# chungongyu/siga

Measured on AMD Instinct MI355X. Metric: reads/sec overlapped (ASQG bit-exact), higher is better.
Workload: dtype u64

## Files before the change

siga_amd/csrc/sigax_kernels.hip:

```cpp
#include <hip/hip_runtime.h>

#include <cstdlib>

#include "sigax_kernels.h"

typedef unsigned long long u64;
typedef unsigned int u32;

#ifndef SIGAX_NT
#define SIGAX_NT 7
#endif

struct Cnt4 {
  u64 a, c, g, t;
};

template <bool WIDE> struct PosOf { typedef u32 type; };
template <> struct PosOf<true> { typedef u64 type; };
template <typename P> struct Cnt4P {
  P a, c, g, t;
};

template <bool WIDE> struct Cand;
template <> struct __attribute__((aligned(32))) Cand<false> {
// ... 170 lines not shown
      "global_load_dwordx4 %3, %9, %12 offset:48\n\t"
      "global_load_dwordx4 %5, %10, %12 offset:16\n\t"
      "global_load_dwordx4 %6, %10, %12 offset:32\n\t"
      "global_load_dwordx4 %7, %10, %12 offset:48\n\t"
      "s_waitcnt vmcnt(0)"
      : "=&v"(a.k0), "=&v"(a.k1), "=&v"(a.k2), "=&v"(a.k3), "=&v"(b.k0), "=&v"(b.k1), "=&v"(b.k2), "=&v"(b.k3), "=&v"(ch)
      : "v"(offa), "v"(offb), "v"(offc), "s"(gbase), "s"(sbase)
      : "memory");
}
__device__ __forceinline__ void find_step_loads8(const void* qa, const void* qb, Gran& a, Gran& b) {
  asm volatile(
      "global_load_dwordx4 %0, %8, off\n\t"
      "global_load_dwordx4 %4, %9, off\n\t"
      "global_load_dwordx4 %1, %8, off offset:16\n\t"
      "global_load_dwordx4 %2, %8, off offset:32\n\t"
      "global_load_dwordx4 %3, %8, off offset:48\n\t"
      "global_load_dwordx4 %5, %9, off offset:16\n\t"
      "global_load_dwordx4 %6, %9, off offset:32\n\t"
      "global_load_dwordx4 %7, %9, off offset:48\n\t"
      "s_waitcnt vmcnt(0)"
      : "=&v"(a.k0), "=&v"(a.k1), "=&v"(a.k2), "=&v"(a.k3), "=&v"(b.k0), "=&v"(b.k1), "=&v"(b.k2), "=&v"(b.k3)
      : "v"(qa), "v"(qb)
      : "memory");
}
__device__ __forceinline__ void find_step_loads8_s(const void* gbase, u32 offa, u32 offb, Gran& a, Gran& b) {
  asm volatile(
      "global_load_dwordx4 %0, %8, %10\n\t"
      "global_load_dwordx4 %4, %9, %10\n\t"
      "global_load_dwordx4 %1, %8, %10 offset:16\n\t"
      "global_load_dwordx4 %2, %8, %10 offset:32\n\t"
      "global_load_dwordx4 %3, %8, %10 offset:48\n\t"
      "global_load_dwordx4 %5, %9, %10 offset:16\n\t"
      "global_load_dwordx4 %6, %9, %10 offset:32\n\t"
      "global_load_dwordx4 %7, %9, %10 offset:48\n\t"
      "s_waitcnt vmcnt(0)"
      : "=&v"(a.k0), "=&v"(a.k1), "=&v"(a.k2), "=&v"(a.k3), "=&v"(b.k0), "=&v"(b.k1), "=&v"(b.k2), "=&v"(b.k3)
      : "v"(offa), "v"(offb), "s"(gbase)
      : "memory");
}
__device__ __forceinline__ void chunk_count(const v4u& k, int take, u32& a, u32& c, u32& g, u32& t) {
  u32 m = take >= 32 ? 0xFFFFFFFFu : (take <= 0 ? 0u : ((1u << take) - 1u));
  u32 x0 = k.y & m, x1 = k.z & m, x2 = k.w & m;
  a += __popc(x0 & ~x1);
  c += __popc(x1 & ~x0);
  g += __popc(x0 & x1);
  t += __popc(x2);
}
template <bool WIDE>
__device__ __forceinline__ Cnt4P<typename PosOf<WIDE>::type> fm_rank4p_from(const FmRef& s, u64 pc, const Gran& q) {
  typedef typename PosOf<WIDE>::type P;
  int r = (int)(pc & 127u);
  u32 a = q.k0.x, c = q.k1.x, g = q.k2.x, t = q.k3.x;
  chunk_count(q.k0, r, a, c, g, t);
  chunk_count(q.k1, r - 32, a, c, g, t);
  chunk_count(q.k2, r - 64, a, c, g, t);
  chunk_count(q.k3, r - 96, a, c, g, t);
  Cnt4P<P> o;
  o.a = a; o.c = c; o.g = g; o.t = t;
  if (WIDE) {
    const u64* sb = s.super + (pc >> SIGAX_SUPER_SHIFT) * 4;
    o.a += (P)sb[0]; o.c += (P)sb[1]; o.g += (P)sb[2]; o.t += (P)sb[3];
  }
  return o;
}

__device__ __forceinline__ u32 fm_char(const FmRef& s, u64 i) {
  const u32* q = reinterpret_cast<const u32*>(s.g) + (i >> 7) * 16 + ((i >> 5) & 3) * 4;
  u32 b = (u32)i & 31u;
  return ((q[1] >> b) & 1u) | (((q[2] >> b) & 1u) << 1) | (((q[3] >> b) & 1u) << 2);
}

__device__ __forceinline__ u32 base_rank(u32 ch) {
  const u32 i = (ch >> 1) & 3u;
  const u32 expect = (0x47544341u >> (i * 8)) & 0xFFu;
  const u32 rank = (0x3421u >> (i * 4)) & 0xFu;
  return expect == ch ? rank : 0u;
}
template <typename T>
__device__ __forceinline__ T sel5(u32 r, T v0, T v1, T v2, T v3, T v4) {
  const bool b0 = (r & 1u) != 0, b1 = (r & 2u) != 0, b2 = (r & 4u) != 0;
  const T t01 = b0 ? v1 : v0, t23 = b0 ? v3 : v2;
  const T t = b1 ? t23 : t01;
  return b2 ? v4 : t;
}
__device__ __forceinline__ u32 comp_rank(u32 r) { return r ? 5u - r : 0u; }

__device__ __forceinline__ u64 wave_sum(u64 v) {
  for (int off = 32; off > 0; off >>= 1) v += __shfl_xor(v, off, 64);
  return v;
}

template <bool WIDE>
__global__ __launch_bounds__(256) void k_occ_batch(FmStrand s, const u64* pos, u64 n, u64* out) {
  u64 i = (u64)blockIdx.x * 256 + threadIdx.x;
  if (i >= n) return;
  u64 v[5];
  fm_rank5<WIDE>(fm_ref(s, 0), pos[i] + 1, v);
  for (int k = 0; k < 5; ++k) out[i * 5 + k] = v[k];
}

template <bool WIDE>
__global__ __launch_bounds__(256) void k_kmer_count(FmStrand s, const unsigned char* kmers, u32 k, u64 n, u64* out) {
  u64 i = (u64)blockIdx.x * 256 + threadIdx.x;
  if (i >= n) return;
  const unsigned char* w = kmers + i * k;
  FmRef f = fm_ref(s, 0);
  u64 C[5] = {s.C[0], s.C[1], s.C[2], s.C[3], s.C[4]};
  u64 T[5] = {s.total[0], s.total[1], s.total[2], s.total[3], s.total[4]};
  auto sel = [](const u64 v[5], u32 r) { return r == 0 ? v[0] : r == 1 ? v[1] : r == 2 ? v[2] : r == 3 ? v[3] : v[4]; };
  u32 r = base_rank(w[k - 1]);
  u64 lo = sel(C, r), hi = lo + sel(T, r) - 1;
  for (u32 j = k - 1; j > 0; --j) {
    if (!(hi != ~0ull && hi >= lo)) break;
    r = base_rank(w[j - 1]);
    u64 l[5], u[5];
    fm_rank5<WIDE>(f, lo, l);
    fm_rank5<WIDE>(f, hi + 1, u);
    lo = sel(C, r) + sel(l, r);
    hi = sel(C, r) + sel(u, r) - 1;
  }
  out[i] = (hi != ~0ull && hi >= lo) ? hi - lo + 1 : 0;
}

template <bool WIDE>
__device__ __forceinline__ u32 lf_row(const FmRef& f, const u64* C, u64 p, u64* next) {
  const u32 c = fm_char(f, p);
  const Cnt4 k = fm_rank<WIDE>(f, p);
  if (c == 0) *next = p - (k.a + k.c + k.g + k.t);
  else *next = C[c] + (c == 1 ? k.a : c == 2 ? k.c : c == 3 ? k.g : k.t);
  return c;
}
#define STRETCH_BAD (~0ull)
template <bool WIDE>
__global__ __launch_bounds__(256) void k_stretch_scan(FmStrand s, u64 n_stretch, u64* info, u32* maxlen) {
  const u64 j = (u64)blockIdx.x * 256 + threadIdx.x;
  u32 mine = 0;
  if (j < n_stretch) {
    const FmRef f = fm_ref(s, 0);
    const u64 C[5] = {s.C[0], s.C[1], s.C[2], s.C[3], s.C[4]};
    u64 p = j, len = 0, v = STRETCH_BAD;
    for (;;) {
      u64 q;
      if (lf_row<WIDE>(f, C, p, &q) == 0) { v = (len << 32) | (q & 0xFFFFFFFFull); break; }
      p = q;
      if (++len >= s.n || len >= (1ull << 28)) { len = 0; break; }
    }
    info[j] = v;
    mine = (u32)len;
  }
  for (int off = 32; off > 0; off >>= 1) mine = max(mine, (u32)__shfl_xor((int)mine, off, 64));
  if ((threadIdx.x & 63u) == 0 && mine) atomicMax(maxlen, mine);
}
__device__ __forceinline__ void packed_or(unsigned char* tab, u64 p, u32 bits, u64 v) {
  const u64 B = p * bits;
  u64* w = reinterpret_cast<u64*>(tab) + (B >> 6);
  const u32 sh = (u32)B & 63u;
  atomicOr(w, v << sh);
  if (sh + bits > 64u) atomicOr(w + 1, v >> (64u - sh));
}
__device__ __forceinline__ u64 packed_get(const unsigned char* tab, u64 p, u32 bits) {
  const u64 B = p * bits;
  u64 v;
#if (SIGAX_NT & 1)
  {
    typedef u64 __attribute__((aligned(1))) u64u;
    v = __builtin_nontemporal_load(reinterpret_cast<const u64u*>(tab + (B >> 3)));
// ... 363 lines not shown
  asm volatile(
      "global_load_dwordx4 %0, %11, %15" SIGAX_FIND_POLICY "\n\t"
      "global_load_dwordx4 %1, %12, %15" SIGAX_FIND_POLICY "\n\t"
      "global_load_dwordx4 %2, %11, %15 offset:80" SIGAX_FIND_POLICY "\n\t"
      "global_load_dwordx4 %3, %11, %15 offset:96" SIGAX_FIND_POLICY "\n\t"
      "global_load_dwordx4 %4, %11, %15 offset:112" SIGAX_FIND_POLICY "\n\t"
      "s_and_saveexec_b64 %10, %16\n\t"
      "global_load_dwordx4 %5, %13, %15" SIGAX_FIND_POLICY "\n\t"
      "global_load_dwordx4 %6, %14, %15" SIGAX_FIND_POLICY "\n\t"
      "global_load_dwordx4 %7, %13, %15 offset:80" SIGAX_FIND_POLICY "\n\t"
      "global_load_dwordx4 %8, %13, %15 offset:96" SIGAX_FIND_POLICY "\n\t"
      "global_load_dwordx4 %9, %13, %15 offset:112" SIGAX_FIND_POLICY "\n\t"
      "s_mov_b64 exec, %10\n\t"
      "s_waitcnt vmcnt(0)"
      : "=&v"(a.s), "=&v"(a.pc), "=&v"(a.p5), "=&v"(a.p6), "=&v"(a.p7), "=&v"(b.s), "=&v"(b.pc), "=&v"(b.p5), "=&v"(b.p6),
        "=&v"(b.p7), "=&s"(saved)
      : "v"(offa), "v"(offa_c), "v"(offb), "v"(offb_c), "s"(base), "s"(two)
      : "memory", "scc");
}
#define COOP_A_U4 512u
#define COOP_B_U4 128u
#define COOP_WAVE_U4 (COOP_A_U4 + COOP_B_U4 + 16u)
__device__ __forceinline__ void find_step2_dma(const uint32_t* gran2, u32 la, u32 lb, u32 c, uint4* stage, u32 lane, Gran2& a, Gran2& b) {
  const u32 j = lane & 7u, pp = lane >> 3;
  const char* base = reinterpret_cast<const char*>(gran2);
  u32* list = reinterpret_cast<u32*>(stage + COOP_A_U4 + COOP_B_U4);
  const bool differ = lb != la;
  const u64 dmask = __ballot(differ);
  const u32 nd = (u32)__popcll(dmask);
  const u32 r = (u32)__popcll(dmask & ((1ull << lane) - 1ull));
  asm volatile("s_waitcnt lgkmcnt(0)" ::: "memory");
  if (differ) list[r] = lb;
#pragma unroll
  for (u32 t = 0; t < 8; ++t) {
    const u32 lA = (u32)__shfl((int)la, (int)(8u * t + j), 64);
    const u32 p = pp ^ (t & 1u);
    const char* sa = base + (u64)lA * 128u + p * 16u;
    __builtin_amdgcn_global_load_lds((const __attribute__((address_space(1))) void*)sa,
                                     (__attribute__((address_space(3))) void*)(u32)(size_t)(stage + t * 64u), 16, 0, 0);
  }
  const u32 tt = lane >> 3, x = tt & 1u;
  auto ld = [](const uint4* q) { const uint4 v = *q; v4u w; w.x = v.x; w.y = v.y; w.z = v.z; w.w = v.w; return w; };
  bool gotA = false;
  const u32 npass = (nd + 15u) >> 4;
  for (u32 ps = 0; ps < npass || !gotA; ++ps) {
    if (ps < npass) {
      asm volatile("s_waitcnt lgkmcnt(0)" ::: "memory");
      __builtin_amdgcn_fence(__ATOMIC_ACQ_REL, "wavefront");
      __builtin_amdgcn_wave_barrier();
#pragma unroll
      for (u32 t = 0; t < 2; ++t) {
        const u32 rk = 16u * ps + 8u * t + j;
        if (rk < nd) {
          const u32 lB = list[rk];
          const u32 p = pp ^ (t & 1u);
          const char* sb = base + (u64)lB * 128u + p * 16u;
          __builtin_amdgcn_global_load_lds((const __attribute__((address_space(1))) void*)sb,
                                           (__attribute__((address_space(3))) void*)(u32)(size_t)(stage + COOP_A_U4 + t * 64u), 16, 0, 0);
        }
      }
    }
    asm volatile("s_waitcnt vmcnt(0)" ::: "memory");
    __builtin_amdgcn_fence(__ATOMIC_ACQUIRE, "wavefront");
    __builtin_amdgcn_wave_barrier();
    if (!gotA) {
      const uint4* qa = stage + tt * 64u + j;
      a.s = ld(qa + ((0u ^ x) * 8u)); a.pc = ld(qa + ((c ^ x) * 8u)); a.p5 = ld(qa + ((5u ^ x) * 8u)); a.p6 = ld(qa + ((6u ^ x) * 8u)); a.p7 = ld(qa + ((7u ^ x) * 8u));
      gotA = true;
    }
    if (differ && (r >> 4) == ps) {
      const u32 q = r & 15u, tb = q >> 3, xb = tb & 1u;
      const uint4* qb = stage + COOP_A_U4 + tb * 64u + (q & 7u);
      b.s = ld(qb + ((0u ^ xb) * 8u)); b.pc = ld(qb + ((c ^ xb) * 8u)); b.p5 = ld(qb + ((5u ^ xb) * 8u)); b.p6 = ld(qb + ((6u ^ xb) * 8u)); b.p7 = ld(qb + ((7u ^ xb) * 8u));
    }
  }
  asm volatile("s_waitcnt lgkmcnt(0)" ::: "memory");
  if (!differ) b = a;
}

struct Rank2 {
  u32 a, c, g, t;
  u32 pa, pc, pg, pt;
};
__device__ __forceinline__ Rank2 rank2_from(const Gran2& q, u32 r, u32 c) {
  const u32 m0 = r >= 32 ? 0xFFFFFFFFu : ((1u << r) - 1u);
  const u32 m1 = r > 32 ? ((1u << (r - 32)) - 1u) : 0u;
  const bool cb0 = ((c - 1u) & 1u) != 0, cb1 = ((c - 1u) & 2u) != 0;
  Rank2 o;
  o.a = q.s.x; o.c = q.s.y; o.g = q.s.z; o.t = q.s.w;
  o.pa = q.pc.x; o.pc = q.pc.y; o.pg = q.pc.z; o.pt = q.pc.w;
  auto word = [&](u32 y, u32 z, u32 w, u32 y2, u32 z2, u32 w2, u32 m) {
    const u32 A = y & ~z, C = z & ~y, G = y & z, T = w;
    o.a += __popc(A & m); o.c += __popc(C & m); o.g += __popc(G & m); o.t += __popc(T & m);
    const u32 E = (cb1 ? (cb0 ? T : G) : (cb0 ? C : A)) & m;
    o.pa += __popc(y2 & ~z2 & E); o.pc += __popc(z2 & ~y2 & E); o.pg += __popc(y2 & z2 & E); o.pt += __popc(w2 & E);
  };
  word(q.p5.x, q.p5.z, q.p6.x, q.p6.z, q.p7.x, q.p7.z, m0);
  word(q.p5.y, q.p5.w, q.p6.y, q.p6.w, q.p7.y, q.p7.w, m1);
  return o;
}
template <bool WIDE>
struct Find2TablesT {
  typedef typename PosOf<WIDE>::type P;
  P Cc[2][4][4];
  P Cd[2][4];
};
typedef Find2TablesT<false> Find2Tables;
template <bool WIDE>
__device__ __forceinline__ void find2_tables_load(Find2TablesT<WIDE>& t, const FmStrand& fwd, const FmStrand& rev) {
  typedef typename PosOf<WIDE>::type P;
  if (threadIdx.x < 8) {
    const u32 which = threadIdx.x >> 2, c = (threadIdx.x & 3u) + 1u;
    const FmStrand& st = which ? rev : fwd;
    const FmRef F = fm_ref(st, which);
    const u64 pos = st.C[c];
    const Cnt4 k = fm_rank<WIDE>(F, pos);
    t.Cc[which][c - 1][0] = (P)k.a; t.Cc[which][c - 1][1] = (P)k.c; t.Cc[which][c - 1][2] = (P)k.g; t.Cc[which][c - 1][3] = (P)k.t;
    t.Cd[which][c - 1] = (P)(pos - (k.a + k.c + k.g + k.t));
  }
}

template <int NT>
struct FindStageT {
  static constexpr bool direct = false;
  uint4 row_[NT][4];
  u64 tag_[NT];
  __device__ __forceinline__ uint4* row(u32 t) { return row_[t]; }
  __device__ __forceinline__ u64& tag(u32 t) { return tag_[t]; }
};
typedef FindStageT<256> FindStage;
typedef FindStageT<128> FindStageC;
struct FindStageNone {
  static constexpr bool direct = true;
  __device__ __forceinline__ uint4* row(u32) { return nullptr; }
  __device__ __forceinline__ u64& tag(u32) { return dummy; }
  u64 dummy;
};

template <class SG>
__device__ __forceinline__ void find_flush(SG& sg, bool want, u32 tid) {
  if constexpr (SG::direct) return;
  const u32 lane = tid & 63u, q0 = tid & ~3u, piece = tid & 3u;
  __builtin_amdgcn_wave_barrier();
  u64 bal = __ballot(want);
  u32 qm = (u32)(bal >> (lane & 60u)) & 0xFu;
  while (__ballot(qm != 0) != 0) {
    if (qm != 0) {
      const u32 src = q0 + (u32)__builtin_ctz(qm);
      const u64 tag = sg.tag(src);
      if (piece <= (u32)(tag & 3u)) {
        const uint4 v = sg.row(src)[piece];
#if (SIGAX_NT & 2)
        {
          typedef u32 nt4 __attribute__((ext_vector_type(4)));
          nt4 w;
          w.x = v.x; w.y = v.y; w.z = v.z; w.w = v.w;
          __builtin_nontemporal_store(w, reinterpret_cast<nt4*>((tag & ~(u64)3) + piece * 16u));
        }
#else
        *reinterpret_cast<uint4*>((tag & ~(u64)3) + piece * 16u) = v;
#endif
      }
      qm &= qm - 1u;
    }
  }
  __builtin_amdgcn_wave_barrier();
}

__device__ __forceinline__ u32 rd_rank(const unsigned char* rd, u32 i) { return ((u32)rd[i >> 1] >> ((i & 1u) * 4u)) & 15u; }

template <bool WIDE, bool STAGED, bool TWO, bool COOP = false, int NT = 256, class SG = FindStage>
__device__ __forceinline__ void find_body(const FindArgs& A, FmTables& tb, SG& sg, const Find2TablesT<WIDE>& t2,
                                          const unsigned char* rd, u64 rd_base, uint4* coop_stage = nullptr, u32 tile = blockIdx.x) {
  const u32 tid = threadIdx.x;
  const u32 wv = __builtin_amdgcn_readfirstlane(tid >> 6);
  const u32 o = A.chain_base + (wv & (A.chains_per_wg - 1u));
  const u32 wslot = (wv / A.chains_per_wg) * 64u + (tid & 63u);
  const u32 slot = A.read_begin + tile * ((u32)NT / A.chains_per_wg) + wslot;
  const bool inr = slot < A.read_end;
  const u32 read = (A.perm != nullptr && inr) ? A.perm[slot] : slot;
  typedef typename PosOf<WIDE>::type P;
  u32 nocc = 0;
  u32 nsec = 0;
  u32 nb = 0, flagbits = 0;
  bool live = inr && ((A.chain_mask >> o) & 1u);
  u64 b0 = 0;
  u32 L = 0;
  if (live) {
    b0 = A.offs[read];
    L = (u32)(A.offs[read + 1] - b0);
    live = L > 0;
  }
  const bool pf = o < 2;
  const FmRef F = fm_ref(A.fwd, 0), R = fm_ref(A.rev, 1);
  const FmRef PI = fm_pick(pf, F, R);
  const FmRef OI = fm_pick(pf, R, F);
  const u64* CP = tb.C[PI.which];
  const u64* CO = tb.C[OI.which];
  const void* PI2 = pf ? (const void*)A.fwd.gran2 : (const void*)A.rev.gran2;
  const u64* PS2 = pf ? A.fwd.super2 : A.rev.super2;
  const bool comp = (o & 1u) != 0;
  const bool fromStart = (o == 1 || o == 2);
  const u32 af = o == 0 ? SIGAX_AF_CHAIN0 : o == 1 ? SIGAX_AF_CHAIN1 : o == 2 ? SIGAX_AF_CHAIN2 : SIGAX_AF_CHAIN3;
  const unsigned char* sq = A.seqs + b0;
  const u32 rdo = A.perm != nullptr ? wslot * A.stage_stride : (u32)(b0 - rd_base);
  const u64 b0w = ((u64)__builtin_amdgcn_readfirstlane((u32)(b0 >> 32)) << 32) | __builtin_amdgcn_readfirstlane((u32)b0);
  const unsigned char* sq0 = A.seqs + b0w;
  const u32 sqd = (u32)(b0 - b0w);
  auto slot_addr = [&](u32 i) -> u64 {
    return reinterpret_cast<u64>(A.arena) + (((u64)read * 4 + o) * A.cap + i) * sizeof(Cand<WIDE>);
  };

  P lo0 = 0, sz = 0, lo1 = 0;
  u32 s = 1;
  bool started = false;
  if (STAGED && A.deep_k != 0u) {
    const u32 K = A.deep_k;
    const bool can = live && L >= K;
    if (__ballot(can) != 0) {
      u64 k0 = 0, k1 = 0;
      bool acgt = can;
      for (u32 i = 0; i < K; ++i) {
        u32 r = 1u;
        if (can) {
          const u32 at = rdo + (fromStart ? i : L - 1u - i);
          r = COOP ? rd_rank(rd, at) : base_rank(rd[at]);
        }
        if (comp) r = comp_rank(r);
        acgt = acgt && r != 0u;
        const u64 c = (u64)((r - 1u) & 3u);
        if (i < 32u) k0 |= c << (2u * i);
        else k1 |= c << (2u * (i - 32u));
      }
      if (acgt) {
        k1 |= (u64)(0x8000u | K) << 48;
        P a0 = 0, a1 = 0, az = 0;
        if (deep_lookup<WIDE>(pf ? A.fwd.deep : A.rev.deep, pf ? A.fwd.deep_slots : A.rev.deep_slots, k0, k1, a0, a1, az)) {
          lo0 = a0; lo1 = a1; sz = az; s = K;
          started = true;
        }
      }
    }
  }
  if (STAGED && live && !started && A.start_ok && L >= (u32)SIGAX_START_K) {
    const void* ST = pf ? A.fwd.start : A.rev.start;
    u32 code = 0;
    bool acgt = true;
#pragma unroll
    for (u32 i = 0; i < (u32)SIGAX_START_K; ++i) {
      const u32 at = rdo + (fromStart ? i : L - 1u - i);
      u32 r = COOP ? rd_rank(rd, at) : base_rank(rd[at]);
      if (comp) r = comp_rank(r);
      acgt = acgt && r != 0u;
      code = (code << 2) | ((r - 1u) & 3u);
    }
    if (acgt) {
      if (WIDE) {
        const ulonglong2* q = reinterpret_cast<const ulonglong2*>(ST) + 2ull * code;
        const ulonglong2 a = q[0], b = q[1];
        lo0 = (P)a.x; lo1 = (P)a.y; sz = (P)b.x; s = (u32)b.y;
      } else {
        const uint4 e = reinterpret_cast<const uint4*>(ST)[code];
        lo0 = (P)e.x; lo1 = (P)e.y; sz = (P)e.z; s = e.w;
      }
      started = true;
    }
  }
  nsec += (u32)__popcll(__ballot(started));
  if (live && !started) {
    u32 r = (STAGED && COOP) ? rd_rank(rd, rdo + (fromStart ? 0 : L - 1)) : base_rank(STAGED ? rd[rdo + (fromStart ? 0 : L - 1)] : sq[fromStart ? 0 : L - 1]);
    if (comp) r = comp_rank(r);
    lo0 = (P)CP[r]; sz = (P)tb.T[PI.which][r]; lo1 = (P)CO[r];
  }
  bool full = !live;
  auto emit = [&](P c0lo, P d, P c1lo, P r0lo, P szv, u32 len) -> bool {
    bool fl = false;
    if constexpr (SG::direct) {
      if (nb < A.cap - 1 && !full) {
        cand_store(reinterpret_cast<Cand<WIDE>*>(slot_addr(nb)), c0lo, d, c1lo, r0lo, c1lo, szv, len, af);
      } else {
        flagbits |= 1u;
        full = true;
      }
      ++nb;
      return false;
    }
    if (nb < A.cap - 1 && !full) {
      if (WIDE) {
        cand_store(reinterpret_cast<Cand<WIDE>*>(sg.row(tid)), c0lo, d, c1lo, r0lo, c1lo, szv, len, af);
        sg.tag(tid) = slot_addr(nb) | 3u;
        fl = true;
      } else {
        cand_store(reinterpret_cast<Cand<WIDE>*>(sg.row(tid) + (nb & 1u) * 2), c0lo, d, c1lo, r0lo, c1lo, szv, len, af);
        if (nb & 1u) {
          sg.tag(tid) = slot_addr(nb - 1) | 3u;
          fl = true;
        }
      }
    } else {
      flagbits |= 1u;
      full = true;
    }
    ++nb;
    return fl;
  };
  for (;;) {
    const bool on = live && sz != 0 && s < L;
    if (__ballot(on) == 0) break;
    if (TWO) {
      u32 c = 0, e = 0;
      const bool want2 = on && s + 1 < L;
      if (want2) {
        if (COOP) {
          c = rd_rank(rd, rdo + (fromStart ? s : L - 1 - s));
          e = rd_rank(rd, rdo + (fromStart ? s + 1 : L - 2 - s));
        } else {
          c = base_rank(rd[rdo + (fromStart ? s : L - 1 - s)]);
          e = base_rank(rd[rdo + (fromStart ? s + 1 : L - 2 - s)]);
        }
        if (comp) { c = comp_rank(c); e = comp_rank(e); }
      }
      const bool ok2 = want2 && c != 0 && e != 0;
      if (__ballot(on && !ok2) == 0) {
        bool fl1 = false, fl2 = false, two_lines = false;
        P lo1n = 0, lo0n = 0, szn = 0, ldn = 0, dd2 = 0, nlo1 = 0, nlo0 = 0, nsz = 0;
        Gran2 ga, gb;
        P pl = 0, pu = 0;
        if (on) {
          const P nn = (P)PI.n;
          pl = lo0 > nn ? nn : lo0;
          const P up = (P)(lo0 + sz);
          pu = (up > nn || up < lo0) ? nn : up;
          two_lines = (pl >> 6) != (pu >> 6);
        }
        const u64 two_mask = COOP ? 0ull : __ballot(two_lines);
        if (COOP) {
          find_step2_dma(reinterpret_cast<const uint32_t*>(PI2), (u32)(pl >> 6), (u32)(pu >> 6), on ? c : 1u,
                         coop_stage + wv * COOP_WAVE_U4, tid & 63u, ga, gb);
        }
        if (on) {
          if (!COOP) {
            const u32 oa = (u32)(pl >> 6) * 128u, ob = (u32)(pu >> 6) * 128u;
            if (A.mask_upper) {
              find_step2_loads_masked(PI2, oa, oa + 16u * c, ob, ob + 16u * c, two_mask, ga, gb);
              if (!two_lines) gb = ga;
            } else {
              find_step2_loads(PI2, oa, oa + 16u * c, ob, ob + 16u * c, ga, gb);
            }
          }
          const Rank2 lr = rank2_from(ga, (u32)pl & 63u, c), ur = rank2_from(gb, (u32)pu & 63u, c);
          P la = lr.a, lcn = lr.c, lg = lr.g, lt = lr.t, ua = ur.a, ucn = ur.c, ug = ur.g, ut = ur.t;
          P lpa = lr.pa, lpc = lr.pc, lpg = lr.pg, lpt = lr.pt, upa = ur.pa, upc = ur.pc, upg = ur.pg, upt = ur.pt;
          if (WIDE) {
            const u64* sl = PS2 + ((u64)pl >> SIGAX_SUPER_SHIFT) * 20;
            const u64* su = PS2 + ((u64)pu >> SIGAX_SUPER_SHIFT) * 20;
            const u32 pb = 4u + (c - 1u) * 4u;
            la += (P)sl[0]; lcn += (P)sl[1]; lg += (P)sl[2]; lt += (P)sl[3];
            ua += (P)su[0]; ucn += (P)su[1]; ug += (P)su[2]; ut += (P)su[3];
            lpa += (P)sl[pb]; lpc += (P)sl[pb + 1]; lpg += (P)sl[pb + 2]; lpt += (P)sl[pb + 3];
            upa += (P)su[pb]; upc += (P)su[pb + 1]; upg += (P)su[pb + 2]; upt += (P)su[pb + 3];
          }
          const P da = ua - la, dc = ucn - lcn, dg = ug - lg, dt = ut - lt;
          const P dd = sz - (da + dc + dg + dt);
          const P ld = lo0 - (la + lcn + lg + lt);
          if (s >= A.minov && dd > 0) fl1 = emit(ld, dd, lo1, lo0, sz, s);
          const P acc1 = sel5<P>(c, (P)0, dd, dd + da, dd + da + dc, dd + da + dc + dg);
          const P lc = sel5<P>(c, ld, la, lcn, lg, lt);
          const P dcc = sel5<P>(c, dd, da, dc, dg, dt);
          lo1n = lo1 + acc1;
          lo0n = (P)CP[c] + lc;
          szn = dcc;
          const P d2a = upa - lpa, d2c = upc - lpc, d2g = upg - lpg, d2t = upt - lpt;
          const P l2d = lc - (lpa + lpc + lpg + lpt);
          dd2 = dcc - (d2a + d2c + d2g + d2t);
          ldn = t2.Cd[PI.which][c - 1] + l2d;
          const P acc2 = sel5<P>(e, (P)0, dd2, dd2 + d2a, dd2 + d2a + d2c, dd2 + d2a + d2c + d2g);
          const P l2e = sel5<P>(e, (P)0, lpa, lpc, lpg, lpt);
          const P d2e = sel5<P>(e, (P)0, d2a, d2c, d2g, d2t);
          nlo1 = lo1n + acc2;
          nlo0 = (P)CP[e] + t2.Cc[PI.which][c - 1][e - 1] + l2e;
          nsz = d2e;
        }
        nsec += 2u * (u32)(__popcll(__ballot(on)) + __popcll(__ballot(two_lines)));
        find_flush(sg, fl1, tid);
        if (on) {
          if (s + 1 >= A.minov && dd2 > 0) fl2 = emit(ldn, dd2, lo1n, lo0n, szn, s + 1);
          lo1 = nlo1; lo0 = nlo0; sz = nsz;
          s += szn != 0 ? 2u : 1u;
        }
        find_flush(sg, fl2, tid);
        continue;
      }
    }
    bool flush = false, two_gran = false;
    if (on) {
      const u64 pl = (u64)lo0 > PI.n ? PI.n : (u64)lo0;
      const u64 pu0 = (u64)(P)(lo0 + sz);
      const u64 pu = pu0 > PI.n ? PI.n : pu0;
      Gran gl, gu;
      u32 ch;
      two_gran = (pl >> 7) != (pu >> 7);
      if (STAGED) {
        ch = COOP ? rd_rank(rd, rdo + (fromStart ? s : L - 1 - s)) : (u32)rd[rdo + (fromStart ? s : L - 1 - s)];
        if (WIDE) find_step_loads8(PI.g + (pl >> 7) * 4, PI.g + (pu >> 7) * 4, gl, gu);
        else find_step_loads8_s(PI.g, (u32)(pl >> 7) * 64u, (u32)(pu >> 7) * 64u, gl, gu);
      } else if (WIDE) {
        find_step_loads(PI.g + (pl >> 7) * 4, PI.g + (pu >> 7) * 4, sq + (fromStart ? s : L - 1 - s), gl, gu, ch);
      } else {
        find_step_loads_s(PI.g, (u32)(pl >> 7) * 64u, (u32)(pu >> 7) * 64u, sq0, sqd + (fromStart ? s : L - 1 - s), gl, gu, ch);
      }
      const Cnt4P<P> l = fm_rank4p_from<WIDE>(PI, pl, gl);
      const Cnt4P<P> u = fm_rank4p_from<WIDE>(PI, pu, gu);
      u32 r = (STAGED && COOP) ? ch : base_rank(ch & 0xFFu);
      if (comp) r = comp_rank(r);
      P da = u.a - l.a, dc = u.c - l.c, dg = u.g - l.g, dt = u.t - l.t;
      P dd = sz - (da + dc + dg + dt);
      const P ld = lo0 - (l.a + l.c + l.g + l.t);
      if (s >= A.minov && dd > 0) flush = emit(ld, dd, lo1, lo0, sz, s);
      const P p1 = dd, p2 = dd + da, p3 = p2 + dc, p4 = p3 + dg;
      const P acc = sel5<P>(r, (P)0, p1, p2, p3, p4);
      const P lc = sel5<P>(r, ld, l.a, l.c, l.g, l.t);
      const P dcur = sel5<P>(r, dd, da, dc, dg, dt);
      lo1 += acc;
      lo0 = (P)CP[r] + lc;
      sz = dcur;
      ++s;
    }
    nsec += (u32)(__popcll(__ballot(on)) + __popcll(__ballot(two_gran)));
    find_flush(sg, flush, tid);
  }
  {
    const bool tail = !WIDE && live && !full && (nb & 1u);
    if (!SG::direct && tail) sg.tag(tid) = slot_addr(nb - 1) | 1u;
    find_flush(sg, tail, tid);
  }
  bool contain = false;
  u32 tail_sec = 0;
  nocc = live ? 2u * (s - 1u) : 0u;
  if (live && sz != 0 && s >= L) {
    auto clampn = [](u64 p, u64 n) { return p > n ? n : p; };
    const u64 pl = clampn((u64)lo0, PI.n), pu = clampn((u64)(P)(lo0 + sz), PI.n);
    const u64 ql = clampn((u64)lo1, OI.n), qu = clampn((u64)(P)(lo1 + sz), OI.n);
    Gran ga, gb;
    u32 ignored;
    tail_sec = ((pl >> 7) != (pu >> 7) ? 2u : 1u) + ((ql >> 7) != (qu >> 7) ? 2u : 1u);
    find_step_loads(PI.g + (pl >> 7) * 4, PI.g + (pu >> 7) * 4, sq, ga, gb, ignored);
    const Cnt4P<P> l = fm_rank4p_from<WIDE>(PI, pl, ga);
    const Cnt4P<P> u = fm_rank4p_from<WIDE>(PI, pu, gb);
    find_step_loads(OI.g + (ql >> 7) * 4, OI.g + (qu >> 7) * 4, sq, ga, gb, ignored);
    const Cnt4P<P> lp = fm_rank4p_from<WIDE>(OI, ql, ga);
    const Cnt4P<P> up = fm_rank4p_from<WIDE>(OI, qu, gb);
    nocc += 4;
    bool dna = (u.a - l.a) | (u.c - l.c) | (u.g - l.g) | (u.t - l.t) | (up.a - lp.a) | (up.c - lp.c) | (up.g - lp.g) |
               (up.t - lp.t);
    if (dna) {
      flagbits |= SIGAX_CC_SUBSTRING;
    } else {
      P ld = lo0 - (l.a + l.c + l.g + l.t);
      P lpd = lo1 - (lp.a + lp.c + lp.g + lp.t);
      if constexpr (SG::direct) {
        cand_store(reinterpret_cast<Cand<WIDE>*>(slot_addr(A.cap - 1)), ld, sz, lpd, lo0, lo1, sz, L, af);
      } else {
        cand_store(reinterpret_cast<Cand<WIDE>*>(sg.row(tid)), ld, sz, lpd, lo0, lo1, sz, L, af);
        sg.tag(tid) = slot_addr(A.cap - 1) | (WIDE ? 3u : 1u);
      }
      flagbits |= SIGAX_CC_CONTAIN;
      contain = true;
    }
  }
  find_flush(sg, contain, tid);
  if (inr) {
    const u32 nbw = (flagbits & 1u) ? 0u : nb;
    u32 word = (nbw & SIGAX_CC_COUNT_MASK) | (flagbits & (SIGAX_CC_SUBSTRING | SIGAX_CC_CONTAIN));
    A.chain_cnt[(u64)read * 4 + o] = word;
  }
  u64 tot_occ = wave_sum((u64)nocc);
  u64 tot_blk = wave_sum((u64)nb + ((flagbits & SIGAX_CC_CONTAIN) ? 1u : 0u));
  u64 tot_err = wave_sum((u64)(flagbits & 1u));
  u64 tot_sec = (u64)nsec + wave_sum((u64)tail_sec);
  u32 mx = nb;
  for (int off = 32; off > 0; off >>= 1) mx = max(mx, (u32)__shfl_xor((int)mx, off, 64));
  if ((threadIdx.x & 63) == 0) {
    if (mx > A.max_seen) atomicMax(&A.dstat[DS_MAX_CHAIN], (u64)mx);
    if (tot_sec) atomicAdd(&A.dstat[DS_SEC_FIND], tot_sec);
    if (tot_occ) atomicAdd(&A.dstat[DS_OCC_FIND], tot_occ);
    if (tot_blk) atomicAdd(&A.dstat[DS_CAND_BLOCKS], tot_blk);
    if (tot_err) atomicAdd(&A.dstat[DS_FIND_OVERFLOW], tot_err);
  }
}

extern __shared__ __attribute__((aligned(16))) unsigned char find_dyn_lds[];
template <int NT = 256>
__device__ __forceinline__ bool find_stage_reads(const FindArgs& A, u64* rd_base) {
  const u32 per = (u32)NT / A.chains_per_wg;
  const u32 r0 = A.read_begin + blockIdx.x * per;
  const u32 r1 = r0 + per < A.read_end ? r0 + per : A.read_end;
  const u64 lo = A.offs[r0], hi = A.offs[r1];
  const u64 alo = (reinterpret_cast<u64>(A.seqs) + lo) & ~3ull;
  const u64 nbytes = reinterpret_cast<u64>(A.seqs) + hi - alo;
  *rd_base = alo - reinterpret_cast<u64>(A.seqs);
  if (nbytes + 4 > (u64)A.stage_bytes) return false;
  const u32* src = reinterpret_cast<const u32*>(alo);
  u32* dst = reinterpret_cast<u32*>(find_dyn_lds);
  const u32 nw = (u32)((nbytes + 3) >> 2);
  for (u32 w = threadIdx.x; w < nw; w += (u32)NT) dst[w] = src[w];
  return true;
}

template <int NT>
__device__ __forceinline__ bool find_stage_reads_perm(const FindArgs& A, u32 tile) {
  const u32 per = (u32)NT / A.chains_per_wg;
  if ((u64)per * A.stage_stride > (u64)A.stage_bytes) return false;
  const u32 r0 = A.read_begin + tile * per;
  const u32 j = threadIdx.x;
  if (j < per && r0 + j < A.read_end) {
    const u32 r = A.perm[r0 + j];
    const u64 b = A.offs[r];
    const u32 len = (u32)(A.offs[r + 1] - b);
    const unsigned char* src = A.seqs + b;
    unsigned char* d = find_dyn_lds + j * A.stage_stride;
    const u32 nw = len >> 2;
    for (u32 k = 0; k < nw; ++k) {
      u32 w;
      __builtin_memcpy(&w, src + 4u * k, 4);
      reinterpret_cast<u32*>(d)[k] = w;
    }
    for (u32 i = nw << 2; i < len; ++i) d[i] = src[i];
  }
  return true;
}

template <int NT>
__device__ __forceinline__ bool find_stage_reads_packed(const FindArgs& A, u64* rd_base, u32 tile) {
  const u32 per = (u32)NT / A.chains_per_wg;
  const u32 r0 = A.read_begin + tile * per;
  const u32 r1 = r0 + per < A.read_end ? r0 + per : A.read_end;
  const u64 lo = A.offs[r0], hi = A.offs[r1];
  const u64 alo = (reinterpret_cast<u64>(A.seqs) + lo) & ~3ull;
  const u64 nbytes = reinterpret_cast<u64>(A.seqs) + hi - alo;
  *rd_base = alo - reinterpret_cast<u64>(A.seqs);
  if ((nbytes + 3) / 2 + 4 > (u64)A.stage_bytes) return false;
  const u32* src = reinterpret_cast<const u32*>(alo);
  unsigned short* dst = reinterpret_cast<unsigned short*>(find_dyn_lds);
  const u32 nw = (u32)((nbytes + 3) >> 2);
  for (u32 w = threadIdx.x; w < nw; w += (u32)NT) {
    const u32 v = src[w];
    dst[w] = (unsigned short)(base_rank(v & 0xFFu) | (base_rank((v >> 8) & 0xFFu) << 4) | (base_rank((v >> 16) & 0xFFu) << 8) |
                              (base_rank(v >> 24) << 12));
  }
  return true;
}

template <int NT>
__device__ __forceinline__ bool find_stage_reads_packed_perm(const FindArgs& A, u32 tile) {
  const u32 per = (u32)NT / A.chains_per_wg;
  if ((u64)per * A.stage_stride / 2u > (u64)A.stage_bytes) return false;
  const u32 r0 = A.read_begin + tile * per;
  const u32 j = threadIdx.x;
  if (j < per && r0 + j < A.read_end) {
    const u32 r = A.perm[r0 + j];
    const u64 b = A.offs[r];
    const u32 len = (u32)(A.offs[r + 1] - b);
    const unsigned char* src = A.seqs + b;
    unsigned char* d = find_dyn_lds + j * (A.stage_stride / 2u);
    const u32 nw = len >> 2;
    for (u32 k = 0; k < nw; ++k) {
      u32 v;
      __builtin_memcpy(&v, src + 4u * k, 4);
      reinterpret_cast<unsigned short*>(d)[k] = (unsigned short)(base_rank(v & 0xFFu) | (base_rank((v >> 8) & 0xFFu) << 4) |
                                                                 (base_rank((v >> 16) & 0xFFu) << 8) | (base_rank(v >> 24) << 12));
    }
    for (u32 i = nw << 2; i < len; ++i) {
      const u32 rk = base_rank(src[i]);
      const u32 old = (i & 1u) ? d[i >> 1] : 0u;
      d[i >> 1] = (unsigned char)((i & 1u) ? ((old & 0x0Fu) | (rk << 4)) : rk);
    }
  }
  return true;
}

__global__ __launch_bounds__(256) __attribute__((amdgpu_waves_per_eu(8, 8))) void k_find_n(FindArgs A) {
  __shared__ FmTables tb;
  __shared__ FindStage sg;
  __shared__ Find2Tables t2;
  u64 rd_base = 0;
  const bool staged = A.perm != nullptr ? find_stage_reads_perm<256>(A, blockIdx.x) : find_stage_reads(A, &rd_base);
  fm_tables_load(tb, A.fwd, A.rev);
  if (staged) find_body<false, true, false>(A, tb, sg, t2, find_dyn_lds, rd_base);
  else find_body<false, false, false>(A, tb, sg, t2, find_dyn_lds, rd_base);
}
__global__ __launch_bounds__(256) void k_find_n2(FindArgs A) {
  __shared__ FmTables tb;
  __shared__ FindStage sg;
  __shared__ Find2Tables t2;
  u64 rd_base = 0;
  const bool staged = A.perm != nullptr ? find_stage_reads_perm<256>(A, blockIdx.x) : find_stage_reads(A, &rd_base);
  find2_tables_load(t2, A.fwd, A.rev);
  fm_tables_load(tb, A.fwd, A.rev);
#ifdef SIGAX_FIND_PRIO
  __builtin_amdgcn_s_setprio(SIGAX_FIND_PRIO);
#endif
  if (staged) find_body<false, true, true>(A, tb, sg, t2, find_dyn_lds, rd_base);
  else find_body<false, false, false>(A, tb, sg, t2, find_dyn_lds, rd_base);
}
__global__ __launch_bounds__(128) void k_find_c2(FindArgs A) {
  __shared__ FmTables tb;
  __shared__ Find2Tables t2;
  __shared__ __attribute__((aligned(16))) uint4 stage[2 * COOP_WAVE_U4];
  find2_tables_load(t2, A.fwd, A.rev);
  fm_tables_load(tb, A.fwd, A.rev);
  const u32 ntiles = (A.read_end - A.read_begin + 63u) / 64u;
  for (u32 tile = blockIdx.x; tile < ntiles; tile += gridDim.x) {
    u64 rd_base = 0;
    const bool staged = A.perm != nullptr ? find_stage_reads_packed_perm<128>(A, tile) : find_stage_reads_packed<128>(A, &rd_base, tile);
    __syncthreads();
    FindStageNone sg;
    if (staged) find_body<false, true, true, true, 128, FindStageNone>(A, tb, sg, t2, find_dyn_lds, rd_base, stage, tile);
    else find_body<false, false, false, false, 128, FindStageNone>(A, tb, sg, t2, find_dyn_lds, rd_base, stage, tile);
    __syncthreads();
  }
}
__global__ __launch_bounds__(128) void k_find_c2w(FindArgs A) {
  __shared__ FmTables tb;
  __shared__ Find2TablesT<true> t2;
  __shared__ __attribute__((aligned(16))) uint4 stage[2 * COOP_WAVE_U4];
  find2_tables_load<true>(t2, A.fwd, A.rev);
  fm_tables_load(tb, A.fwd, A.rev);
  const u32 ntiles = (A.read_end - A.read_begin + 63u) / 64u;
  for (u32 tile = blockIdx.x; tile < ntiles; tile += gridDim.x) {
    u64 rd_base = 0;
    const bool staged = A.perm != nullptr ? find_stage_reads_packed_perm<128>(A, tile) : find_stage_reads_packed<128>(A, &rd_base, tile);
    __syncthreads();
    FindStageNone sg;
    if (staged) find_body<true, true, true, true, 128, FindStageNone>(A, tb, sg, t2, find_dyn_lds, rd_base, stage, tile);
    else find_body<true, false, false, false, 128, FindStageNone>(A, tb, sg, t2, find_dyn_lds, rd_base, stage, tile);
    __syncthreads();
  }
}
__global__ __launch_bounds__(256) void k_find_w(FindArgs A) {
  __shared__ FmTables tb;
  __shared__ FindStage sg;
  __shared__ Find2TablesT<true> t2;
  u64 rd_base = 0;
  const bool staged = A.perm != nullptr ? find_stage_reads_perm<256>(A, blockIdx.x) : find_stage_reads(A, &rd_base);
  fm_tables_load(tb, A.fwd, A.rev);
  if (staged) find_body<true, true, false>(A, tb, sg, t2, find_dyn_lds, rd_base);
  else find_body<true, false, false>(A, tb, sg, t2, find_dyn_lds, rd_base);
}

#define FX_COUNTDOWN 0x80000000u
struct Ent {
  u64 c0lo, c0hi, c1lo, c1hi;
  u32 src, len;
  u32 pad0, pad1;
};

__device__ __forceinline__ bool iv_valid(u64 lo, u64 hi) { return hi != ~0ull && hi >= lo; }
__device__ __forceinline__ bool intersecting(u64 s1, u64 e1, u64 s2, u64 e2) { return !(s1 > e2 || s2 > e1); }

template <bool WIDE>
struct Fx {
  const FxArgs& A;
  const FmTables& tb;
  FmRef F, R;
  Ent* pool;
  u32 top;
  bool overflow;
  bool xerror;
  u64 nocc;
  u32 read, nout;
  const Cand<WIDE>* slots;

  __device__ Fx(const FxArgs& a, const FmTables& t, Ent* p)
      : A(a), tb(t), F(fm_ref(a.fwd, 0)), R(fm_ref(a.rev, 1)), pool(p), top(0), overflow(false), xerror(false), nocc(0),
        read(0), nout(0), slots(nullptr) {}

  __device__ u32 af_of(u32 src) const {
    u32 ch = src / A.cap;
    return ch == 0 ? SIGAX_AF_CHAIN0 : ch == 1 ? SIGAX_AF_CHAIN1 : ch == 2 ? SIGAX_AF_CHAIN2 : SIGAX_AF_CHAIN3;
  }
  __device__ FmRef ext_index(u32 src) const { return fm_pick((src / A.cap) < 2, R, F); }

  __device__ bool need(u32 upto) {
    if (upto + nout > A.pool_cap) { overflow = true; return false; }
    return true;
// ... 2432 lines not shown
```

Before: 153.3 million.

## Precompute base ranks in staged LDS reads and simplify rank2 symbol masking

In k_find_n2, reads are converted to rank bytes while being staged into LDS. Each byte holds the forward rank in the low nibble and the complement rank in the high nibble, so the hot backward-search loop can fetch ranks with a shift-and-mask instead of base_rank/comp_rank per character. rank2_from now builds branch-free masks and selects the extension symbol with XOR-based bit masks instead of nested selects, and sel5 is replaced by a 4-way sel4 for known nonzero ranks. find_flush also returns early when no lane needs to flush. This adds ALU work during staging and depends on the nibble encoding being correct on every path.

```diff
diff --git a/siga_amd/csrc/sigax_kernels.hip b/siga_amd/csrc/sigax_kernels.hip
--- a/siga_amd/csrc/sigax_kernels.hip
+++ b/siga_amd/csrc/sigax_kernels.hip
@@ -276,6 +276,11 @@
   const T t01 = b0 ? v1 : v0, t23 = b0 ? v3 : v2;
   const T t = b1 ? t23 : t01;
   return b2 ? v4 : t;
+}
+template <typename T>
+__device__ __forceinline__ T sel4(u32 r, T v1, T v2, T v3, T v4) {
+  const bool b0 = ((r - 1u) & 1u) != 0, b1 = ((r - 1u) & 2u) != 0;
+  return b1 ? (b0 ? v4 : v3) : (b0 ? v2 : v1);
 }
 __device__ __forceinline__ u32 comp_rank(u32 r) { return r ? 5u - r : 0u; }
 
@@ -805,23 +810,30 @@
   u32 a, c, g, t;
   u32 pa, pc, pg, pt;
 };
-__device__ __forceinline__ Rank2 rank2_from(const Gran2& q, u32 r, u32 c) {
-  const u32 m0 = r >= 32 ? 0xFFFFFFFFu : ((1u << r) - 1u);
-  const u32 m1 = r > 32 ? ((1u << (r - 32)) - 1u) : 0u;
-  const bool cb0 = ((c - 1u) & 1u) != 0, cb1 = ((c - 1u) & 2u) != 0;
+struct SymMask {
+  u32 y, z, w;
+};
+__device__ __forceinline__ SymMask sym_mask(u32 c) {
+  SymMask k;
+  k.y = 0u - (c & 1u); k.z = 0u - ((c >> 1) & 1u); k.w = 0u - ((c >> 2) & 1u);
+  return k;
+}
+__device__ __forceinline__ Rank2 rank2_from(const Gran2& q, u32 r, const SymMask& k) {
+  const u32 f = (1u << (r & 31u)) - 1u, h = 0u - ((r >> 5) & 1u);
+  const u32 m0 = f | h, m1 = f & h;
   Rank2 o;
   o.a = q.s.x; o.c = q.s.y; o.g = q.s.z; o.t = q.s.w;
   o.pa = q.pc.x; o.pc = q.pc.y; o.pg = q.pc.z; o.pt = q.pc.w;
   auto word = [&](u32 y, u32 z, u32 w, u32 y2, u32 z2, u32 w2, u32 m) {
-    const u32 A = y & ~z, C = z & ~y, G = y & z, T = w;
-    o.a += __popc(A & m); o.c += __popc(C & m); o.g += __popc(G & m); o.t += __popc(T & m);
-    const u32 E = (cb1 ? (cb0 ? T : G) : (cb0 ? C : A)) & m;
+    o.a += __popc(y & ~z & m); o.c += __popc(z & ~y & m); o.g += __popc(y & z & m); o.t += __popc(w & m);
+    const u32 E = ~(w ^ k.w) & ~(z ^ k.z) & ~((y ^ k.y) | ~m);
     o.pa += __popc(y2 & ~z2 & E); o.pc += __popc(z2 & ~y2 & E); o.pg += __popc(y2 & z2 & E); o.pt += __popc(w2 & E);
   };
   word(q.p5.x, q.p5.z, q.p6.x, q.p6.z, q.p7.x, q.p7.z, m0);
   word(q.p5.y, q.p5.w, q.p6.y, q.p6.w, q.p7.y, q.p7.w, m1);
   return o;
 }
+__device__ __forceinline__ Rank2 rank2_from(const Gran2& q, u32 r, u32 c) { return rank2_from(q, r, sym_mask(c)); }
 template <bool WIDE>
 struct Find2TablesT {
   typedef typename PosOf<WIDE>::type P;
@@ -865,7 +877,11 @@
   if constexpr (SG::direct) return;
   const u32 lane = tid & 63u, q0 = tid & ~3u, piece = tid & 3u;
   __builtin_amdgcn_wave_barrier();
-  u64 bal = __ballot(want);
+  const u64 bal = __ballot(want);
+  if (bal == 0) {
+    __builtin_amdgcn_wave_barrier();
+    return;
+  }
   u32 qm = (u32)(bal >> (lane & 60u)) & 0xFu;
   while (__ballot(qm != 0) != 0) {
     if (qm != 0) {
@@ -892,7 +908,7 @@
 
 __device__ __forceinline__ u32 rd_rank(const unsigned char* rd, u32 i) { return ((u32)rd[i >> 1] >> ((i & 1u) * 4u)) & 15u; }
 
-template <bool WIDE, bool STAGED, bool TWO, bool COOP = false, int NT = 256, class SG = FindStage>
+template <bool WIDE, bool STAGED, bool TWO, bool COOP = false, int NT = 256, class SG = FindStage, bool RB = false>
 __device__ __forceinline__ void find_body(const FindArgs& A, FmTables& tb, SG& sg, const Find2TablesT<WIDE>& t2,
                                           const unsigned char* rd, u64 rd_base, uint4* coop_stage = nullptr, u32 tile = blockIdx.x) {
   const u32 tid = threadIdx.x;
@@ -925,6 +941,12 @@
   const bool comp = (o & 1u) != 0;
   const bool fromStart = (o == 1 || o == 2);
   const u32 af = o == 0 ? SIGAX_AF_CHAIN0 : o == 1 ? SIGAX_AF_CHAIN1 : o == 2 ? SIGAX_AF_CHAIN2 : SIGAX_AF_CHAIN3;
+  const u32 csh = comp ? 4u : 0u;
+  auto staged_rank = [&](u32 at) -> u32 {
+    if (RB) return ((u32)rd[at] >> csh) & 15u;
+    const u32 r = COOP ? rd_rank(rd, at) : base_rank(rd[at]);
+    return comp ? comp_rank(r) : r;
+  };
   const unsigned char* sq = A.seqs + b0;
   const u32 rdo = A.perm != nullptr ? wslot * A.stage_stride : (u32)(b0 - rd_base);
   const u64 b0w = ((u64)__builtin_amdgcn_readfirstlane((u32)(b0 >> 32)) << 32) | __builtin_amdgcn_readfirstlane((u32)b0);
@@ -945,11 +967,7 @@
       bool acgt = can;
       for (u32 i = 0; i < K; ++i) {
         u32 r = 1u;
-        if (can) {
-          const u32 at = rdo + (fromStart ? i : L - 1u - i);
-          r = COOP ? rd_rank(rd, at) : base_rank(rd[at]);
-        }
-        if (comp) r = comp_rank(r);
+        if (can) r = staged_rank(rdo + (fromStart ? i : L - 1u - i));
         acgt = acgt && r != 0u;
         const u64 c = (u64)((r - 1u) & 3u);
         if (i < 32u) k0 |= c << (2u * i);
@@ -971,9 +989,7 @@
     bool acgt = true;
 #pragma unroll
     for (u32 i = 0; i < (u32)SIGAX_START_K; ++i) {
-      const u32 at = rdo + (fromStart ? i : L - 1u - i);
-      u32 r = COOP ? rd_rank(rd, at) : base_rank(rd[at]);
-      if (comp) r = comp_rank(r);
+      const u32 r = staged_rank(rdo + (fromStart ? i : L - 1u - i));
       acgt = acgt && r != 0u;
       code = (code << 2) | ((r - 1u) & 3u);
     }
@@ -991,8 +1007,13 @@
   }
   nsec += (u32)__popcll(__ballot(started));
   if (live && !started) {
-    u32 r = (STAGED && COOP) ? rd_rank(rd, rdo + (fromStart ? 0 : L - 1)) : base_rank(STAGED ? rd[rdo + (fromStart ? 0 : L - 1)] : sq[fromStart ? 0 : L - 1]);
-    if (comp) r = comp_rank(r);
+    u32 r;
+    if (STAGED) {
+      r = staged_rank(rdo + (fromStart ? 0 : L - 1));
+    } else {
+      r = base_rank(sq[fromStart ? 0 : L - 1]);
+      if (comp) r = comp_rank(r);
+    }
     lo0 = (P)CP[r]; sz = (P)tb.T[PI.which][r]; lo1 = (P)CO[r];
   }
   bool full = !live;
@@ -1034,19 +1055,24 @@
       u32 c = 0, e = 0;
       const bool want2 = on && s + 1 < L;
       if (want2) {
-        if (COOP) {
+        if (RB) {
+          const u32 at = rdo + (fromStart ? s : L - 2 - s);
+          const u32 w = (u32)rd[at] | ((u32)rd[at + 1] << 8);
+          c = (w >> (csh + (fromStart ? 0u : 8u))) & 15u;
+          e = (w >> (csh + (fromStart ? 8u : 0u))) & 15u;
+        } else if (COOP) {
           c = rd_rank(rd, rdo + (fromStart ? s : L - 1 - s));
           e = rd_rank(rd, rdo + (fromStart ? s + 1 : L - 2 - s));
         } else {
           c = base_rank(rd[rdo + (fromStart ? s : L - 1 - s)]);
           e = base_rank(rd[rdo + (fromStart ? s + 1 : L - 2 - s)]);
         }
-        if (comp) { c = comp_rank(c); e = comp_rank(e); }
+        if (comp && !RB) { c = comp_rank(c); e = comp_rank(e); }
       }
       const bool ok2 = want2 && c != 0 && e != 0;
       if (__ballot(on && !ok2) == 0) {
         bool fl1 = false, fl2 = false, two_lines = false;
-        P lo1n = 0, lo0n = 0, szn = 0, ldn = 0, dd2 = 0, nlo1 = 0, nlo0 = 0, nsz = 0;
+        P lo1n, lo0n, szn, ldn, dd2, nlo1, nlo0, nsz;
         Gran2 ga, gb;
         P pl = 0, pu = 0;
         if (on) {
@@ -1071,7 +1097,8 @@
               find_step2_loads(PI2, oa, oa + 16u * c, ob, ob + 16u * c, ga, gb);
             }
           }
-          const Rank2 lr = rank2_from(ga, (u32)pl & 63u, c), ur = rank2_from(gb, (u32)pu & 63u, c);
+          const SymMask km = sym_mask(c);
+          const Rank2 lr = rank2_from(ga, (u32)pl & 63u, km), ur = rank2_from(gb, (u32)pu & 63u, km);
           P la = lr.a, lcn = lr.c, lg = lr.g, lt = lr.t, ua = ur.a, ucn = ur.c, ug = ur.g, ut = ur.t;
           P lpa = lr.pa, lpc = lr.pc, lpg = lr.pg, lpt = lr.pt, upa = ur.pa, upc = ur.pc, upg = ur.pg, upt = ur.pt;
           if (WIDE) {
@@ -1087,9 +1114,9 @@
           const P dd = sz - (da + dc + dg + dt);
           const P ld = lo0 - (la + lcn + lg + lt);
           if (s >= A.minov && dd > 0) fl1 = emit(ld, dd, lo1, lo0, sz, s);
-          const P acc1 = sel5<P>(c, (P)0, dd, dd + da, dd + da + dc, dd + da + dc + dg);
-          const P lc = sel5<P>(c, ld, la, lcn, lg, lt);
-          const P dcc = sel5<P>(c, dd, da, dc, dg, dt);
+          const P acc1 = sel4<P>(c, dd, dd + da, dd + da + dc, dd + da + dc + dg);
+          const P lc = sel4<P>(c, la, lcn, lg, lt);
+          const P dcc = sel4<P>(c, da, dc, dg, dt);
           lo1n = lo1 + acc1;
           lo0n = (P)CP[c] + lc;
           szn = dcc;
@@ -1097,9 +1124,9 @@
           const P l2d = lc - (lpa + lpc + lpg + lpt);
           dd2 = dcc - (d2a + d2c + d2g + d2t);
           ldn = t2.Cd[PI.which][c - 1] + l2d;
-          const P acc2 = sel5<P>(e, (P)0, dd2, dd2 + d2a, dd2 + d2a + d2c, dd2 + d2a + d2c + d2g);
-          const P l2e = sel5<P>(e, (P)0, lpa, lpc, lpg, lpt);
-          const P d2e = sel5<P>(e, (P)0, d2a, d2c, d2g, d2t);
+          const P acc2 = sel4<P>(e, dd2, dd2 + d2a, dd2 + d2a + d2c, dd2 + d2a + d2c + d2g);
+          const P l2e = sel4<P>(e, lpa, lpc, lpg, lpt);
+          const P d2e = sel4<P>(e, d2a, d2c, d2g, d2t);
           nlo1 = lo1n + acc2;
           nlo0 = (P)CP[e] + t2.Cc[PI.which][c - 1][e - 1] + l2e;
           nsz = d2e;
@@ -1134,8 +1161,13 @@
       }
       const Cnt4P<P> l = fm_rank4p_from<WIDE>(PI, pl, gl);
       const Cnt4P<P> u = fm_rank4p_from<WIDE>(PI, pu, gu);
-      u32 r = (STAGED && COOP) ? ch : base_rank(ch & 0xFFu);
-      if (comp) r = comp_rank(r);
+      u32 r;
+      if (RB) {
+        r = (ch >> csh) & 15u;
+      } else {
+        r = (STAGED && COOP) ? ch : base_rank(ch & 0xFFu);
+        if (comp) r = comp_rank(r);
+      }
       P da = u.a - l.a, dc = u.c - l.c, dg = u.g - l.g, dt = u.t - l.t;
       P dd = sz - (da + dc + dg + dt);
       const P ld = lo0 - (l.a + l.c + l.g + l.t);
@@ -1212,8 +1244,16 @@
   }
 }
 
+__device__ __forceinline__ u32 rank_byte(u32 ch) {
+  const u32 r = base_rank(ch);
+  return r | (comp_rank(r) << 4);
+}
+__device__ __forceinline__ u32 rank_bytes4(u32 v) {
+  return rank_byte(v & 0xFFu) | (rank_byte((v >> 8) & 0xFFu) << 8) | (rank_byte((v >> 16) & 0xFFu) << 16) | (rank_byte(v >> 24) << 24);
+}
+
 extern __shared__ __attribute__((aligned(16))) unsigned char find_dyn_lds[];
-template <int NT = 256>
+template <int NT = 256, bool RB = false>
 __device__ __forceinline__ bool find_stage_reads(const FindArgs& A, u64* rd_base) {
   const u32 per = (u32)NT / A.chains_per_wg;
   const u32 r0 = A.read_begin + blockIdx.x * per;
@@ -1226,11 +1266,11 @@
   const u32* src = reinterpret_cast<const u32*>(alo);
   u32* dst = reinterpret_cast<u32*>(find_dyn_lds);
   const u32 nw = (u32)((nbytes + 3) >> 2);
-  for (u32 w = threadIdx.x; w < nw; w += (u32)NT) dst[w] = src[w];
+  for (u32 w = threadIdx.x; w < nw; w += (u32)NT) dst[w] = RB ? rank_bytes4(src[w]) : src[w];
   return true;
 }
 
-template <int NT>
+template <int NT, bool RB = false>
 __device__ __forceinline__ bool find_stage_reads_perm(const FindArgs& A, u32 tile) {
   const u32 per = (u32)NT / A.chains_per_wg;
   if ((u64)per * A.stage_stride > (u64)A.stage_bytes) return false;
@@ -1246,9 +1286,9 @@
     for (u32 k = 0; k < nw; ++k) {
       u32 w;
       __builtin_memcpy(&w, src + 4u * k, 4);
-      reinterpret_cast<u32*>(d)[k] = w;
-    }
-    for (u32 i = nw << 2; i < len; ++i) d[i] = src[i];
+      reinterpret_cast<u32*>(d)[k] = RB ? rank_bytes4(w) : w;
+    }
+    for (u32 i = nw << 2; i < len; ++i) d[i] = (unsigned char)(RB ? rank_byte(src[i]) : src[i]);
   }
   return true;
 }
@@ -1317,13 +1357,13 @@
   __shared__ FindStage sg;
   __shared__ Find2Tables t2;
   u64 rd_base = 0;
-  const bool staged = A.perm != nullptr ? find_stage_reads_perm<256>(A, blockIdx.x) : find_stage_reads(A, &rd_base);
+  const bool staged = A.perm != nullptr ? find_stage_reads_perm<256, true>(A, blockIdx.x) : find_stage_reads<256, true>(A, &rd_base);
   find2_tables_load(t2, A.fwd, A.rev);
   fm_tables_load(tb, A.fwd, A.rev);
 #ifdef SIGAX_FIND_PRIO
   __builtin_amdgcn_s_setprio(SIGAX_FIND_PRIO);
 #endif
-  if (staged) find_body<false, true, true>(A, tb, sg, t2, find_dyn_lds, rd_base);
+  if (staged) find_body<false, true, true, false, 256, FindStage, true>(A, tb, sg, t2, find_dyn_lds, rd_base);
   else find_body<false, false, false>(A, tb, sg, t2, find_dyn_lds, rd_base);
 }
 __global__ __launch_bounds__(128) void k_find_c2(FindArgs A) {
```

Result: no change. 152.6 million, median of 2 (-0.5%).
